# indrajeetadityaroy9/vit-inductive-bias-distillation

Measured on AMD Instinct MI355X. Metric: distillation images/sec (BASD loss fwd+bwd+grad all-reduce), DeiT-S<-ResNet-50 @ bs256/GPU, higher is better.
Workload: dtype f32; 1 GPU; cfg2 DeiT-S<-ResNet-50 224x224; per_gpu_batch=256, global_batch=256, input_dtype=float32, layout=strided (CLS-sliced / channel-major views), backward=True, grad_allreduce_bytes=88202672, grad_allreduce=none at world size 1 (bucket packed, nothing to exchange), rank_readback=auto, readback_deferred_steps=1756, selector=basd_selector_chain mode 0, parallelism=dp1

## Files before the change

### include/basd_hip.h

```cpp
#ifndef BASD_HIP_H
#define BASD_HIP_H

#include <stdint.h>

#ifdef __cplusplus
extern "C" {
#endif

#ifndef __HIP_PLATFORM_AMD__
typedef struct ihipStream_t* hipStream_t;
#endif

#define BASD_OK 0
#define BASD_EINVAL (-1)
#define BASD_EUNSUPPORTED (-2)
#define BASD_DTYPE_F32 0
#define BASD_DTYPE_BF16 1
#define BASD_DTYPE_U8 2


int basd_gemm_nt(const void* a, int a_dtype, long a_sb, long a_sn, long a_sd, int a_rows_per_batch,
                 long a_batch_stride, const float* b, long ldb, long b_batch_stride, int M, int N, int K, int batch,
                 float* c, long ldc, long c_batch_stride, float scale, const float* bias, float beta,
                 float* colsum_part, float* col_mean, hipStream_t stream);

int basd_gemm_tn_splits(int krows);

int basd_gemm_tn(const void* a, const void* b, int dtype, long a_sb, long a_sn, long a_sd, long a_batch_stride,
                 long b_sb, long b_sn, long b_sd, long b_batch_stride, int rows_per_batch, int krows, int M, int N,
                 int batch, const float* mean_a, const float* mean_b, int splits, float* slabs, float* c, long ldc,
                 long c_batch_stride, float scale, hipStream_t stream);

int basd_colmean_parts(int rows);

int basd_colmean(const void* x, int dtype, long sb, long sn, long sd, int rows_per_batch, long batch_stride,
                 int rows, int cols, int batch, int parts, float* partial, float* mean, hipStream_t stream);

int basd_gemm_tuning(int split_bf16);
int basd_gemm_tuning_get(void);

int basd_colmean_multi(const void* const* x_ptrs, int dtype, long sb, long sn, long sd, int rows_per_batch, int rows,
                       int cols, int n_mats, int parts, float* partial, float* means, int vec_ok,
                       hipStream_t stream);

int basd_syrk_splits(int krows, int cols, int n_mats);

int basd_syrk_multi(const void* const* x_ptrs, int dtype, long sb, long sn, long sd, int rows_per_batch, int krows,
                    int cols, int n_mats, const float* means, const float* scales, int splits, float* slabs,
                    float* out, long out_stride, int vec_ok, const float* fold, int fold_parts, int fold_from,
                    hipStream_t stream);


int basd_jacobi_workspace_ints(int batch, int max_sweeps);
int basd_jacobi_max_rows(void);
int basd_jacobi_plain4_fits(int n);

int basd_jacobi_tuning(int lanes_per_pair);
int basd_jacobi_ordering(int odd_even);

int basd_jacobi_onesided(float* W, long batch_stride, int rows_dot, int rows_tot, int n, int batch,
                         const int* n_arr, float* colnorm, int colnorm_stride, int max_sweeps, float tol_cos,
                         int* flags, int* sweeps_out, hipStream_t stream);
int basd_jacobi_plan_query(int rows_dot, int rows_tot, int n, int batch, int per_matrix_orders, int* out8);

long basd_jacobi_twopass_workspace_bytes(int n, int batch, int max_sweeps);
int basd_jacobi_stacked_twopass(float* W, long batch_stride, int n, int batch, float* colnorm, int colnorm_stride,
                                int max_sweeps, float tol_cos, void* workspace, int* sweeps_out, hipStream_t stream);

int basd_sort_extract(const float* W, long batch_stride, int rows, int rows_tot, int n, int batch,
                      const float* colnorm, int colnorm_stride, float* vals_desc, float* vecs, int kmax,
                      hipStream_t stream);


long basd_tridiag_workspace_bytes(int n, int batch);

int basd_tridiag(float* a, long a_batch_stride, int n, int batch, float* d, float* e, float* tau, float* vh,
                 void* work, hipStream_t stream);

int basd_tridiag_ranked(float* a, long a_batch_stride, int n, int batch, float* d, float* e, float* tau, float* vh,
                        void* work, int rank_count, double factor, int cap, int* rank_out, int* host_mirror,
                        void* mid_event ,
                        hipStream_t stream);

// ... 410 lines not shown
```

### vit-inductive-bias-distillation_amd/basd_amd/_lib.py

```python
from __future__ import annotations

import ctypes as C
import os
import threading

_HERE = os.path.dirname(os.path.abspath(__file__))
LIB_PATH = os.path.join(_HERE, "libbasd_hip.so")

vp, i32, i64, f32, f64 = C.c_void_p, C.c_int, C.c_long, C.c_float, C.c_double

SIGNATURES = {
    "basd_gemm_nt": [vp, i32, i64, i64, i64, i32, i64, vp, i64, i64, i32, i32, i32, i32, vp, i64, i64, f32, vp, f32,
                     vp, vp, vp],
    "basd_gemm_tn_splits": [i32],
    "basd_gemm_tn": [vp, vp, i32, i64, i64, i64, i64, i64, i64, i64, i64, i32, i32, i32, i32, i32, vp, vp, i32, vp,
                     vp, i64, i64, f32, vp],
    "basd_colmean_parts": [i32],
    "basd_colmean": [vp, i32, i64, i64, i64, i32, i64, i32, i32, i32, i32, vp, vp, vp],
    "basd_colmean_multi": [vp, i32, i64, i64, i64, i32, i32, i32, i32, i32, vp, vp, i32, vp],
    "basd_syrk_splits": [i32, i32, i32],
    "basd_syrk_multi": [vp, i32, i64, i64, i64, i32, i32, i32, i32, vp, vp, i32, vp, vp, i64, i32, vp, i32, i32, vp],
    "basd_jacobi_workspace_ints": [i32, i32],
    "basd_jacobi_max_rows": [],
    "basd_jacobi_twopass_workspace_bytes": [i32, i32, i32],
    "basd_jacobi_stacked_twopass": [vp, i64, i32, i32, vp, i32, i32, f32, vp, vp, vp],
    "basd_jacobi_tuning": [i32],
    "basd_jacobi_ordering": [i32],
    "basd_gemm_tuning": [i32],
    "basd_gemm_tuning_get": [],
    "basd_jacobi_onesided": [vp, i64, i32, i32, i32, i32, vp, vp, i32, i32, f32, vp, vp, vp],
    "basd_jacobi_plan_query": [i32, i32, i32, i32, i32, vp],
    "basd_sort_extract": [vp, i64, i32, i32, i32, i32, vp, i32, vp, vp, i32, vp],
    "basd_tridiag_workspace_bytes": [i32, i32],
    "basd_tridiag_tuning": [i32, i32, i32, i32, i32, i32],
    "basd_tridiag": [vp, i64, i32, i32, vp, vp, vp, vp, vp, vp],
    "basd_tridiag_ranked": [vp, i64, i32, i32, vp, vp, vp, vp, vp, i32, f64, i32, vp, vp, vp, vp],
    "basd_tridiag_ranked_gated": [vp, i64, i32, i32, vp, vp, vp, vp, vp, i32, f64, i32, vp, vp, vp, C.c_uint, i32, vp],
    "basd_flag_set": [vp, C.c_uint, vp],
    "basd_scale_unless_one": [vp, i64, vp, vp, vp],
    "basd_event_create": [vp],
    "basd_event_destroy": [vp],
    "basd_stream_wait_event": [vp, vp],
    "basd_tridiag_eigenvalues": [vp, vp, i32, i32, vp, vp],
    "basd_tridiag_eigenvalues_leading": [vp, vp, i32, i32, i32, vp, vp],
    "basd_tridiag_apply_q": [vp, vp, i32, i32, i32, vp, vp, i32, i32, vp],
    "basd_tridiag_shifted_solve": [vp, vp, vp, i32, i32, i32, i32, vp, vp, vp],
    "basd_tridiag_mp_rank": [vp, vp, i32, i32, f64, i32, vp, vp, vp, vp, vp],
    "basd_tridiag_mp_rank_rank1": [vp, vp, vp, i32, i32, f64, f64, i32, vp, vp, vp, vp],
    "basd_tridiag_eigenvectors": [vp, vp, vp, vp, vp, i32, i32, i32, vp, vp, i32, vp],
    "basd_mp_rank": [vp, i32, i32, f64, i32, vp, vp, vp],
    "basd_grassmann_distance": [vp, i32, vp, vp, i32, vp, i32, vp, vp, vp],
    "basd_grassmann_distance_padded": [vp, i32, i32, vp, vp, i32, vp, i32, vp, vp],
    "basd_selector_tail": [vp] * 10 + [i32, i32, i32, i32] + [vp] * 14 + [vp],
    "basd_sqrt_clamp": [vp, vp, i64, vp],
# ... 164 lines not shown
```

### vit-inductive-bias-distillation_amd/csrc/chain.hip

```cpp
#include "basd_common.h"
#include "../../include/basd_hip.h"
#include <stdlib.h>

namespace basd {

__global__ void __launch_bounds__(256) chain_sw_kernel(const float* __restrict__ vals, int n, int kmax,
                                                       float* __restrict__ sw) {
    const int l = blockIdx.x;
    for (int i = threadIdx.x; i < kmax; i += 256) sw[(long)l * kmax + i] = sqrtf(fmaxf(vals[(long)l * n + i], 0.f));
}

__global__ void chain_k_arr_kernel(const int* __restrict__ ranks, int L, int items, int kmax, int* __restrict__ k_arr) {
    const int i = blockIdx.x * blockDim.x + threadIdx.x;
    if (i < items) {
        int k = ranks[i % L];
        k = k < 1 ? 1 : k;
        k_arr[i] = k > kmax ? kmax : k;
    }
}

constexpr int CERT_BLOCKS = 32;
__global__ void __launch_bounds__(256) rank_certificate_kernel(const float* __restrict__ grams, const float* __restrict__ zbar,
                                                               int n, int L, double factor, double* __restrict__ scratch,
                                                               int* __restrict__ host_flag) {
    __shared__ double part[2][4];
    __shared__ int s_last;
    const int tid = threadIdx.x, lane = tid & 63, wave = tid >> 6, l = blockIdx.y;
    const long nn = (long)n * n;
    const float* g = grams + l * nn;
    double s2 = 0.0, tr = 0.0;
    for (long idx = (long)blockIdx.x * 256 + tid; idx < nn; idx += (long)CERT_BLOCKS * 256) {
        const double v = (double)g[idx];
        s2 = fma(v, v, s2);
    }
    if (blockIdx.x == 0)
        for (int i = tid; i < n; i += 256) tr += (double)g[(long)i * n + i];
    for (int off = 32; off > 0; off >>= 1) {
        s2 += __shfl_down(s2, off, 64);
        tr += __shfl_down(tr, off, 64);
    }
    if (lane == 0) { part[0][wave] = s2; part[1][wave] = tr; }
    __syncthreads();
    int* ticket = (int*)(scratch + 4L * L);
    if (tid == 0) {
        atomicAdd(scratch + 4 * l + 0, part[0][0] + part[0][1] + part[0][2] + part[0][3]);
        if (blockIdx.x == 0) atomicAdd(scratch + 4 * l + 1, part[1][0] + part[1][1] + part[1][2] + part[1][3]);
        __threadfence();
        s_last = atomicAdd(ticket, 1) == CERT_BLOCKS * L - 1;
    }
    __syncthreads();
    if (!s_last) return;
    __threadfence();
    __shared__ int s_ok;
    if (tid == 0) s_ok = 1;
    __syncthreads();
    for (int m = wave; m < L; m += 4) {
        double zz = 0.0;
        if (zbar)
            for (int i = lane; i < n; i += 64) {
                const double z = (double)zbar[(long)m * n + i];
                zz = fma(z, z, zz);
            }
        for (int off = 32; off > 0; off >>= 1) zz += __shfl_down(zz, off, 64);
        if (lane == 0) {
            const double a = __hip_atomic_load(scratch + 4 * m + 0, __ATOMIC_RELAXED, __HIP_MEMORY_SCOPE_AGENT);
            const double b = __hip_atomic_load(scratch + 4 * m + 1, __ATOMIC_RELAXED, __HIP_MEMORY_SCOPE_AGENT);
            const double c = (double)(n - (n - 1) / 2);
            bool good = false;
            if (b > 0.0 && c > 1.0) {
                const double lo = fmax(zz, a / b);
                const double tr_a = fmax(b - zz, 1e-4 * b);
                const double hi = fmin(b / c, tr_a / (c - 1.0));
                good = lo > 1.5 * factor * hi;
            }
            if (!good) atomicAnd(&s_ok, 0);
            scratch[4 * m + 0] = 0.0;
            scratch[4 * m + 1] = 0.0;
        }
    }
    __syncthreads();
    if (tid == 0) {
        *ticket = 0;
        *host_flag = s_ok;
        __threadfence_system();
    }
}

__global__ void __launch_bounds__(256) chain_mask_cos_kernel(float* __restrict__ cos, int kmax, const int* __restrict__ k_arr) {
    const int k = k_arr[blockIdx.x];
    float* c = cos + (long)blockIdx.x * kmax * kmax;
    for (int idx = threadIdx.x; idx < kmax * kmax; idx += 256) {
        const int i = idx / kmax, j = idx - i * kmax;
        if (i >= k || j >= k) c[idx] = 0.f;
    }
// ... 131 lines not shown
    if (M_t < n || M_t > 0x7fffffff || M_s > 0x7fffffff) return BASD_EUNSUPPORTED;
    const long nn = (long)n * n;
    const int tiles = (int)((M_t + 127) / 128);
    hipStream_t cs = a->chain_stream, ss = a->student_stream;

    if (a->main_stream) BASD_HIP(hipEventRecord((hipEvent_t)a->ev_fork, a->main_stream));
    BASD_HIP(hipStreamWaitEvent(cs, (hipEvent_t)a->ev_fork, 0));
    if (ss != cs) BASD_HIP(hipStreamWaitEvent(ss, (hipEvent_t)a->ev_fork, 0));
    if (a->ev_slot_free) {
        BASD_HIP(hipStreamWaitEvent(cs, (hipEvent_t)a->ev_slot_free, 0));
        if (ss != cs) BASD_HIP(hipStreamWaitEvent(ss, (hipEvent_t)a->ev_slot_free, 0));
    }

    const bool early = mode == 3 && a->go_flag != nullptr && a->fact_stream != nullptr && a->go_value != 0;
    if (early) {
        hipStream_t fs = a->fact_stream;
        if (a->ev_slot_free) BASD_HIP(hipStreamWaitEvent(fs, (hipEvent_t)a->ev_slot_free, 0));
        int rc_early = basd_tridiag_ranked_gated(a->grams, nn, n, 2 * L, a->d, a->e, a->tau, a->vh, a->tri_work, L,
                                                 a->mp_factor, (int)a->rank_cap, a->ranks, a->host_mirror, a->go_flag,
                                                 (unsigned)a->go_value, (int)a->go_budget, fs);
        if (rc_early != BASD_OK) return rc_early;
        BASD_HIP(hipEventRecord((hipEvent_t)a->ev_ranks, fs));
    }
    for (int l = 0; l < L; ++l)
        BASD_TRY(basd_gemm_nt(a->teacher_host_ptrs[l], (int)a->t_dtype, a->t_sb, a->t_sn, a->t_sd, n_t, 0, a->proj_t, d_t,
                              0, (int)M_t, n, d_t, 1, a->z + (long)l * M_t * n, n, M_t * n, 1.f, nullptr, 0.f,
                              a->z_sums + (long)l * tiles * n, a->z_means + (long)l * n, cs));
    BASD_MARK(a->tm_proj, cs);
    if (mode == 4) {
        BASD_CHECK_ARG(a->ev_tgram != nullptr && ss != cs);
        BASD_HIP(hipEventRecord((hipEvent_t)a->ev_tgram, cs));
        BASD_HIP(hipStreamWaitEvent(ss, (hipEvent_t)a->ev_tgram, 0));
    }
    BASD_TRY(basd_syrk_multi(a->z_ptrs, BASD_DTYPE_F32, 0, n, 1, 1 << 30, (int)M_t, n, L, a->z_means, nullptr,
                             (int)a->t_splits, a->t_slabs, a->grams + (long)L * nn, nn, 1, nullptr, 0, 0, cs));
    BASD_TRY(basd_gram_finish(a->grams + (long)L * nn, a->z_means, n, L, M_t, a->grams, nullptr, cs));
    BASD_MARK(a->tm_tgram, cs);
    if (mode == 3) BASD_CHECK_ARG(a->ev_tg0 != nullptr);
    if (a->ev_tg0) BASD_HIP(hipEventRecord((hipEvent_t)a->ev_tg0, cs));
    if (a->cert_mirror) {
        BASD_CHECK_ARG(a->cert_stream && a->ev_cert && a->ev_tg0 && a->cert_scratch);
        if (a->cert_stream != cs) BASD_HIP(hipStreamWaitEvent(a->cert_stream, (hipEvent_t)a->ev_tg0, 0));
        BASD_TRY(basd_rank_certificate(a->grams, a->z_means, n, L, a->mp_factor, a->cert_scratch, a->cert_mirror, a->cert_stream));
        BASD_HIP(hipEventRecord((hipEvent_t)a->ev_cert, a->cert_stream));
    }

    auto student_grams = [&](hipStream_t st) -> int {
        BASD_MARK(a->tm_scol0, st);
        BASD_TRY(basd_colmean_multi(a->student_ptrs, (int)a->s_dtype, a->s_sb, a->s_sn, a->s_sd, n_s, (int)M_s, n, E,
                                    (int)a->s_parts, a->s_partial, a->s_means, (int)a->s_vec_ok, st));
        BASD_MARK(a->tm_scol1, st);
        BASD_TRY(basd_syrk_multi(a->student_ptrs, (int)a->s_dtype, a->s_sb, a->s_sn, a->s_sd, n_s, (int)M_s, n, E,
                                 a->s_means, nullptr, (int)a->s_splits, a->s_slabs, a->grams + 2L * L * nn, nn,
                                 (int)a->s_vec_ok, nullptr, 0, 0, st));
        BASD_MARK(a->tm_sgram, st);
        return BASD_OK;
    };

    if (mode == 0 || mode == 4) {
        BASD_TRY(student_grams(ss));
        if (ss != cs) {
            BASD_HIP(hipEventRecord((hipEvent_t)a->ev_student, ss));
            BASD_HIP(hipStreamWaitEvent(cs, (hipEvent_t)a->ev_student, 0));
        }
        BASD_MARK(a->tm_tri0, cs);
        BASD_TRY(basd_tridiag_ranked(a->grams, nn, n, 2 * L + E, a->d, a->e, a->tau, a->vh, a->tri_work, L, a->mp_factor,
                                     (int)a->rank_cap, a->ranks, a->host_mirror, a->tm_mid, cs));
        BASD_HIP(hipEventRecord((hipEvent_t)a->ev_ranks, cs));
    } else {
// ... 26 lines not shown
```

### vit-inductive-bias-distillation_amd/csrc/gemm.hip

```cpp
#include <type_traits>

#include "basd_common.h"

namespace basd {

typedef float f32x16 __attribute__((ext_vector_type(16)));
typedef float f32x4 __attribute__((ext_vector_type(4)));

template <typename T>
using lds_ptr = const __attribute__((address_space(3))) T*;

constexpr int BM = 128, BN = 128;

typedef __bf16 bf16x8 __attribute__((ext_vector_type(8)));

__device__ __forceinline__ unsigned cvt_pk_bf16(float a, float b) {
    unsigned r;
    asm("v_cvt_pk_bf16_f32 %0, %1, %2" : "=v"(r) : "v"(a), "v"(b));
    return r;
}

__device__ __forceinline__ void split3(float a, float b, unsigned& hi, unsigned& mid, unsigned& lo) {
    hi = cvt_pk_bf16(a, b);
    const float ra = a - __uint_as_float(hi << 16), rb = b - __uint_as_float(hi & 0xffff0000u);
// ... 646 lines not shown
    syrk_grid_decode(splits * n_mats, pairs, pair, unit);
    int tmi, tni;
    tri_tile(pair, tmi, tni);
    const bool diag = tmi == tni;
    lds_t* tA = lds;
    lds_t* tB = diag ? lds : lds + Path::TN_TILE;
    const int tid = threadIdx.x, lane = tid & 63, wave = tid >> 6, wm = wave >> 1, wn = wave & 1;
    const int m0 = tmi * BM, n0 = tni * BN;
    const int z = unit / splits, sp = unit - z * splits;
    X.ptr = ptrs[z];
    const float* mean = means ? means + (long)z * cols : nullptr;
    float* C = slabs + ((long)z * splits + sp) * (long)cols * cols;
    int k_begin, k_end;
    tn_split_range(Krows, splits, sp, k_begin, k_end);

    f32x16 acc[2][2];
    zero_acc(acc);

    const bool is_b = tid >= 128;
    const bool loader = !(is_b && diag);
    const int t = tid & 127;
    const int col0 = is_b ? n0 : m0;
    float m4[4];
    TnCursor cu;
    tn_cursor_init(cu, X, k_begin, t);
    if (fold && z >= fold_from)
        tn_fold_mean4(fold + (long)(z - fold_from) * fold_parts * cols, fold_parts, cols, Krows, col0, t, m4);
    else
        tn_mean4(mean, cols, col0, t, m4);
    tn_main_loop<Path, T, VEC>(X, cu, loader, k_begin, k_end, cols, col0, t, m4, is_b ? tB : tA, tA, tB, wm, wn, lane, acc);
    Path::tn_store_c(C, cols, cols, cols, m0, n0, acc, wm, wn, lane, 1.f);
}

__global__ void __launch_bounds__(256) syrk_reduce_kernel(const float* __restrict__ slabs, int cols, int splits,
                                                          const float* __restrict__ scales, float* __restrict__ out,
                                                          long out_stride) {
    int tmi, tni;
    tri_tile(blockIdx.x >> 6, tmi, tni);
    const int e = (blockIdx.x & 63) * 256 + threadIdx.x;
    const int r = tmi * BM + (e >> 7), c = tni * BN + (e & 127);
    if (r >= cols || c >= cols) return;
    const int z = blockIdx.y;
    const long mat = (long)cols * cols;
    const bool up = tmi == tni && r < c;
    const float* in = slabs + (long)z * splits * mat + (up ? (long)c * cols + r : (long)r * cols + c);
    float s = 0.f;
    for (int k = 0; k < splits; ++k) s += in[k * mat];
    s *= scales ? scales[z] : 1.f;
    float* o = out + (long)z * out_stride;
    o[(long)r * cols + c] = s;
    if (tmi != tni) o[(long)c * cols + r] = s;
}

__global__ void reduce_slabs_kernel(const float* __restrict__ slabs, long slab_stride, int splits, long count,
                                    float scale, float* __restrict__ out, long batch_in_stride,
                                    long batch_out_stride) {
    const float* in = slabs + (long)blockIdx.y * batch_in_stride;
    float* o = out + (long)blockIdx.y * batch_out_stride;
    for (long i = (long)blockIdx.x * blockDim.x + threadIdx.x; i < count; i += (long)gridDim.x * blockDim.x) {
        float s = 0.f;
        for (int k = 0; k < splits; ++k) s += in[(long)k * slab_stride + i];
        o[i] = s * scale;
    }
}

template <typename T>
__global__ void __launch_bounds__(256) colsum_partial_kernel(GemmOperand X, int rows, int cols, int parts,
                                                             float* __restrict__ partial,
                                                             const void* const* __restrict__ ptrs = nullptr) {
    __shared__ float red[4][64];
    const int cl = threadIdx.x & 63, rg = threadIdx.x >> 6, c = blockIdx.x * 64 + cl;
    const T* base = ptrs ? (const T*)ptrs[blockIdx.z] : (const T*)X.ptr + (long)blockIdx.z * X.batch_stride;
    const int per = (rows + parts - 1) / parts;
    const int r0 = blockIdx.y * per, r1 = min(rows, r0 + per);
    float s = 0.f;
    if (c < cols)
        for (int r = r0 + rg; r < r1; r += 4) s += to_f32(base[row_off(X, r) + (long)c * X.sd]);
    red[rg][cl] = s;
    __syncthreads();
    if (rg == 0 && c < cols)
        partial[((long)blockIdx.z * parts + blockIdx.y) * cols + c] = (red[0][cl] + red[1][cl]) + (red[2][cl] + red[3][cl]);
}

__device__ __forceinline__ float4 load4(const float* p) { return *(const float4*)p; }
// ... 192 lines not shown
    BASD_CHECK_ARG(x && partial && mean && rows > 0 && cols > 0 && batch > 0 && parts >= 1);
    GemmOperand X{x, sb, sn, sd, rows_per_batch, batch_stride};
    const int esz = dtype == BASD_DTYPE_F32 ? 4 : 2;
    const bool vec = sd == 1 && cols % 4 == 0 && ((uintptr_t)x & 15) == 0 && (sb * esz) % 16 == 0 &&
                     (sn * esz) % 16 == 0 && (batch_stride * esz) % 16 == 0;
    if (dtype == BASD_DTYPE_F32) launch_colsum<float>(X, nullptr, x, rows, cols, parts, batch, vec, partial, stream);
    else if (dtype == BASD_DTYPE_BF16) launch_colsum<__hip_bfloat16>(X, nullptr, x, rows, cols, parts, batch, vec, partial, stream);
    else return BASD_EINVAL;
    colsum_final_kernel<<<dim3((cols + 63) / 64, batch), 256, 0, stream>>>(partial, cols, parts, 1.f / rows, mean);
    BASD_RETURN_LAST();
}

int basd_syrk_splits(int krows, int cols, int n_mats) {
    const int tiles = (cols + BM - 1) / BM, pairs = tiles * (tiles + 1) / 2;
    const long w = (long)pairs * n_mats;
    const int chunks = (krows + TN_BK - 1) / TN_BK;
    int cap = chunks / 8;
    if (cap > 64) cap = 64;
    if (cap < 1) cap = 1;
    const double slots = 768.0;
    auto fill = [&](int s) {
        const double x = (double)(w * s) / slots;
        const double rounds = x <= 1.0 ? 1.0 : (double)(long)(x + 0.999999);
        return x / rounds;
    };
    double best_eff = 0.0;
    for (int s = 1; s <= cap; ++s) best_eff = fill(s) > best_eff ? fill(s) : best_eff;
    int best = cap;
    for (int s = 1; s <= cap; ++s)
        if (fill(s) >= 0.97 * best_eff) { best = s; break; }
    return best;
}

int basd_syrk_multi(const void* const* x_ptrs, int dtype, long sb, long sn, long sd, int rows_per_batch, int krows,
                    int cols, int n_mats, const float* means, const float* scales, int splits, float* slabs,
                    float* out, long out_stride, int vec_ok, const float* fold, int fold_parts, int fold_from,
                    hipStream_t stream) {
    BASD_CHECK_ARG(x_ptrs && slabs && out && krows > 0 && cols > 0 && n_mats > 0 && splits >= 1 && rows_per_batch > 0);
    BASD_CHECK_ARG(out_stride >= (long)cols * cols);
    BASD_CHECK_ARG(!fold || (fold_parts > 0 && fold_from >= 0 && fold_from <= n_mats));
    GemmOperand X{nullptr, sb, sn, sd, rows_per_batch, 0};
    const int tiles = (cols + BM - 1) / BM, pairs = tiles * (tiles + 1) / 2;
    const dim3 grid(pairs * splits * n_mats);
    const bool vec = dtype == BASD_DTYPE_F32 ? vec_ok && sd == 1 && sb % 4 == 0 && sn % 4 == 0 : sd == 1;
    const bool known = dispatch_mfma(g_gemm_split, dtype, vec, [&](auto path, auto el, auto v) {
        syrk_tn_kernel<decltype(path), typename decltype(el)::type, decltype(v)::value><<<grid, 256, 0, stream>>>(
            x_ptrs, X, cols, krows, splits, n_mats, pairs, means, slabs, fold, fold_parts, fold_from);
    });
    if (!known) return BASD_EINVAL;
    syrk_reduce_kernel<<<dim3(pairs * 64, n_mats), 256, 0, stream>>>(slabs, cols, splits, scales, out, out_stride);
    BASD_RETURN_LAST();
}

int basd_colmean_multi(const void* const* x_ptrs, int dtype, long sb, long sn, long sd, int rows_per_batch, int rows,
                       int cols, int n_mats, int parts, float* partial, float* means, int vec_ok,
                       hipStream_t stream) {
    BASD_CHECK_ARG(x_ptrs && partial && means && rows > 0 && cols > 0 && n_mats > 0 && parts >= 1);
    GemmOperand X{nullptr, sb, sn, sd, rows_per_batch, 0};
    const int esz = dtype == BASD_DTYPE_F32 ? 4 : 2;
    const bool vec = vec_ok && sd == 1 && cols % 4 == 0 && (sb * esz) % 16 == 0 && (sn * esz) % 16 == 0;
    if (dtype == BASD_DTYPE_F32) launch_colsum<float>(X, x_ptrs, nullptr, rows, cols, parts, n_mats, vec, partial, stream);
    else if (dtype == BASD_DTYPE_BF16) launch_colsum<__hip_bfloat16>(X, x_ptrs, nullptr, rows, cols, parts, n_mats, vec, partial, stream);
    else return BASD_EINVAL;
    colsum_final_kernel<<<dim3((cols + 63) / 64, n_mats), 256, 0, stream>>>(partial, cols, parts, 1.f / rows, means);
    BASD_RETURN_LAST();
}

}
```

### vit-inductive-bias-distillation_amd/csrc/procrustes.hip

```cpp
#include "basd_common.h"
#include "../../include/basd_hip.h"

namespace basd {

typedef double f64x4 __attribute__((ext_vector_type(4)));

template <typename T>
__global__ void __launch_bounds__(256) token_weights_kernel(const void* const* __restrict__ attn_ptrs,
                                                            const float* __restrict__ mix, int L, long sb, long sh,
                                                            long sq, long sk, int H, int A, int has_cls, int n_a,
                                                            int n_t, int n_s, const int* __restrict__ atap0,
                                                            const int* __restrict__ atap1,
                                                            const float* __restrict__ alam,
                                                            const int* __restrict__ tap0,
                                                            const int* __restrict__ tap1,
                                                            const float* __restrict__ lam, float* __restrict__ omega,
                                                            float* __restrict__ omega_t, float* __restrict__ raw_out) {
    extern __shared__ float sm[];
    float* raw = sm;
    float* w = sm + n_a;
    __shared__ float red[32];
    const int b = blockIdx.x, tid = threadIdx.x;
    for (int j = tid; j < n_a; j += blockDim.x) {
        float acc = 0.f;
        if (has_cls) {
            for (int h = 0; h < H; ++h) {
                float m = 0.f;
                for (int l = 0; l < L; ++l)
                    m += mix[l] * ldg_f32((const BASD_GLOBAL_AS T*)attn_ptrs[l] + (b * sb + h * sh + (long)(1 + j) * sk));
                acc += m;
            }
            acc /= (float)H;
        } else {
            for (int h = 0; h < H; ++h)
                for (int q = 0; q < A; ++q) {
                    float m = 0.f;
                    for (int l = 0; l < L; ++l)
                        m += mix[l] * ldg_f32((const BASD_GLOBAL_AS T*)attn_ptrs[l] + (b * sb + h * sh + q * sq + (long)j * sk));
                    acc += m;
                }
            acc /= (float)(H * A);
        }
        raw[j] = acc;
        if (raw_out) raw_out[(long)b * n_a + j] = acc;
    }
    __syncthreads();
    float part = 0.f;
    for (int n = tid; n < n_s; n += blockDim.x) {
        float v;
        if (atap0) {
            const float l1 = alam[n];
            v = (1.f - l1) * raw[atap0[n]] + l1 * raw[atap1[n]];
        } else {
            v = raw[n];
        }
        w[n] = v;
        part += v;
    }
    const float total = block_sum(part, red);
    for (int n = tid; n < n_s; n += blockDim.x) {
        const float v = w[n] / total;
        w[n] = v;
        omega[(long)b * n_s + n] = v;
    }
    __syncthreads();
    for (int j = tid; j < n_t; j += blockDim.x) {
        float acc = 0.f;
        if (tap0) {
            for (int n = 0; n < n_s; ++n) {
                const float l1 = lam[n];
                if (tap0[n] == j) acc += (1.f - l1) * w[n];
                if (tap1[n] == j) acc += l1 * w[n];
            }
        } else {
            acc = w[j];
        }
        omega_t[(long)b * n_t + j] = acc;
    }
}

template <typename T>
__global__ void __launch_bounds__(256) student_project_kernel(const T* __restrict__ X, long sb, long sn, int n_s,
                                                              int n_t, int D, const float* __restrict__ omega,
                                                              const int* __restrict__ tap0,
                                                              const int* __restrict__ tap1,
                                                              const float* __restrict__ lam,
                                                              const int* __restrict__ range0,
                                                              const int* __restrict__ range1,
                                                              float* __restrict__ mu_out, float* __restrict__ tr_part,
                                                              float* __restrict__ Ap) {
    extern __shared__ float sm[];
    float* w = sm;
    __shared__ float red[4][64];
    __shared__ float mu[64];
    __shared__ float scratch[32];
    const int b = blockIdx.y, d0 = blockIdx.x * 64, tid = threadIdx.x;
    const int cl = tid & 63, rg = tid >> 6, d = d0 + cl;
    const bool live = d < D;
    const T* Xb = X + (long)b * sb + d;
    for (int n = tid; n < n_s; n += 256) w[n] = omega[(long)b * n_s + n];
    __syncthreads();
    float acc = 0.f;
    if (live)
        for (int n = rg; n < n_s; n += 4) acc = fmaf(w[n], to_f32(Xb[(long)n * sn]), acc);
    red[rg][cl] = acc;
// ... 168 lines not shown
    if (tid < SP_W) {
        float m = 0.f;
#pragma unroll
        for (int q = 0; q < 32; ++q) m += red[q][tid];
        mu[tid] = m;
        if (d0 + tid < D) mu_out[((long)e * B + b) * D + d0 + tid] = m;
    }
    __syncthreads();
    const float4 m4 = *(const float4*)(mu + c4);
    float part = 0.f;
    if (live)
        for (int n = rg; n < n_s; n += 32) {
            const float4 v = *(const float4*)(xs + n * SP_W + c4);
            const float cx = v.x - m4.x, cy = v.y - m4.y, cz = v.z - m4.z, cw = v.w - m4.w;
            part = fmaf(w[n], fmaf(cx, cx, fmaf(cy, cy, fmaf(cz, cz, cw * cw))), part);
        }
    const float tr = block_sum(part, scratch);
    if (tid == 0) tr_part[((long)e * B + b) * gridDim.x + blockIdx.x] = tr;
    if (!live) return;
    float* Ab = Ap + ((long)e * B + b) * n_t * D + d0 + c4;
    for (int j = rg; j < n_t; j += 32) {
        const int n0 = range0 ? range0[j] : j, n1 = range1 ? range1[j] : j + 1;
        float4 a = make_float4(0.f, 0.f, 0.f, 0.f);
        for (int n = n0; n < n1; ++n) {
            const float cw = tap0 ? (t0[n] == j ? c0[n] : 0.f) + (t1[n] == j ? c1[n] : 0.f) : w[n];
            const float4 v = *(const float4*)(xs + n * SP_W + c4);
            a.x = fmaf(cw, v.x - m4.x, a.x); a.y = fmaf(cw, v.y - m4.y, a.y);
            a.z = fmaf(cw, v.z - m4.z, a.z); a.w = fmaf(cw, v.w - m4.w, a.w);
        }
        *(float4*)(Ab + (long)j * D) = a;
    }
}

template <typename T>
__global__ void __launch_bounds__(256) teacher_center_kernel(const void* const* __restrict__ tok_ptrs,
                                                             const float* __restrict__ mix, int L, long sb, long sn,
                                                             long sd, int n, int D, const int* __restrict__ g0,
                                                             const int* __restrict__ g1,
                                                             const float* __restrict__ glam,
                                                             const float* __restrict__ omega_t,
                                                             float* __restrict__ mu_out, float* __restrict__ Tc) {
    extern __shared__ float sm[];
    float* tile = sm;
    float* wt = sm + (size_t)n * 65;
    float* mu = wt + n;
    const int b = blockIdx.y, d0 = blockIdx.x * 64, tid = threadIdx.x;
    for (int j = tid; j < n; j += 256) wt[j] = omega_t[(long)b * n + j];
    const int total = n * 64;
    const bool feat_fast = sd == 1;
    for (int idx = tid; idx < total; idx += 256) {
        int j, dd;
        if (feat_fast) { j = idx >> 6; dd = idx & 63; }
        else { dd = idx / n; j = idx - dd * n; }
        const int d = d0 + dd;
        float v = 0.f;
        if (d < D) {
            const long off = b * sb + (long)d * sd;
            if (g0) {
                const long r0 = g0[j], r1 = g1[j];
                float a0 = 0.f, a1 = 0.f;
                for (int l = 0; l < L; ++l) {
                    const BASD_GLOBAL_AS T* p = (const BASD_GLOBAL_AS T*)tok_ptrs[l];
                    a0 = fmaf(mix[l], ldg_f32(p + (off + r0 * sn)), a0);
                    a1 = fmaf(mix[l], ldg_f32(p + (off + r1 * sn)), a1);
                }
                const float l1 = glam[j];
                v = (1.f - l1) * a0 + l1 * a1;
            } else {
                for (int l = 0; l < L; ++l)
                    v = fmaf(mix[l], ldg_f32((const BASD_GLOBAL_AS T*)tok_ptrs[l] + (off + (long)j * sn)), v);
            }
        }
        tile[j * 65 + dd] = v;
    }
    __syncthreads();
    if (tid < 64) {
        float acc = 0.f;
        for (int j = 0; j < n; ++j) acc = fmaf(wt[j], tile[j * 65 + tid], acc);
        mu[tid] = acc;
        if (d0 + tid < D) mu_out[(long)b * D + d0 + tid] = acc;
    }
    __syncthreads();
    float* out = Tc + (long)b * n * D;
    for (int idx = tid; idx < total; idx += 256) {
        const int j = idx >> 6, dd = idx & 63, d = d0 + dd;
        if (d < D) out[(long)j * D + d] = tile[j * 65 + dd] - mu[dd];
    }
}

constexpr int TCM_W = 16, TCM_G = 4;
template <typename T>
__global__ void __launch_bounds__(256) teacher_center_multi_kernel(
    const void* const* __restrict__ tok_ptrs, const float* __restrict__ mix, int L, int G, long sb, long sn, long sd,
    int n, int D, const int* __restrict__ g0, const int* __restrict__ g1, const float* __restrict__ glam,
    const float* __restrict__ omega_t, float* __restrict__ mu_out, float* __restrict__ Tc) {
    extern __shared__ float sm[];
    const int B = gridDim.y, b = blockIdx.y, d0 = blockIdx.x * TCM_W, tid = threadIdx.x;
    float* tile = sm;
    float* wt = sm + (size_t)G * n * (TCM_W + 1);
    float* mu = wt + (size_t)G * n;
    for (int idx = tid; idx < G * n; idx += 256) {
        const int g = idx / n, j = idx - g * n;
        wt[idx] = omega_t[((long)g * B + b) * n + j];
    }
    const int total = n * TCM_W;
    const bool feat_fast = sd == 1;
    for (int idx = tid; idx < total; idx += 256) {
// ... 945 lines not shown
                                                                      const int* __restrict__ tap0,
                                                                      const int* __restrict__ tap1,
                                                                      const float* __restrict__ lam,
                                                                      const int* __restrict__ range0,
                                                                      const int* __restrict__ range1,
                                                                      float* __restrict__ dX) {
    const int j = blockIdx.x, b = blockIdx.y;
    const int s0 = range0[j], s1 = range1[j];
    for (int d = threadIdx.x; d < D; d += 128) {
        float acc = 0.f;
        for (int s = s0; s < s1; ++s) {
            const float l1 = lam[s];
            const float coef = (tap0[s] == j ? 1.f - l1 : 0.f) + (tap1[s] == j ? l1 : 0.f);
            acc = fmaf(coef, dY[((long)b * n_out + s) * D + d], acc);
        }
        dX[((long)b * n_in + j) * D + d] = acc;
    }
}

}

using namespace basd;

extern "C" {

int basd_token_weights(const void* const* attn_ptrs, int dtype, const float* mix, int L, long sb, long sh, long sq,
                       long sk, int B, int H, int A, int has_cls, int n_a, int n_t, int n_s, const int* atap0,
                       const int* atap1, const float* alam, const int* tap0, const int* tap1, const float* lam,
                       float* omega, float* omega_t, float* raw_out, hipStream_t stream) {
    BASD_CHECK_ARG(attn_ptrs && mix && omega && omega_t && L > 0 && B > 0 && H > 0 && n_a > 0 && n_t > 0 && n_s > 0);
    BASD_CHECK_ARG(A == n_a + (has_cls ? 1 : 0));
    BASD_CHECK_ARG((n_a == n_s) == (atap0 == nullptr));
    BASD_CHECK_ARG((n_t == n_s) == (tap0 == nullptr));
    const size_t lds = sizeof(float) * (size_t)(n_a + n_s);
    if (dtype == BASD_DTYPE_F32)
        token_weights_kernel<float><<<B, 256, lds, stream>>>(attn_ptrs, mix, L, sb, sh, sq, sk, H, A, has_cls, n_a, n_t, n_s, atap0, atap1, alam, tap0, tap1, lam, omega, omega_t, raw_out);
    else if (dtype == BASD_DTYPE_BF16)
        token_weights_kernel<__hip_bfloat16><<<B, 256, lds, stream>>>(attn_ptrs, mix, L, sb, sh, sq, sk, H, A, has_cls, n_a, n_t, n_s, atap0, atap1, alam, tap0, tap1, lam, omega, omega_t, raw_out);
    else
        return BASD_EINVAL;
    BASD_RETURN_LAST();
}

int basd_student_project(const void* x, int dtype, long sb, long sn, int B, int n_s, int n_t, int D,
                         const float* omega, const int* tap0, const int* tap1, const float* lam, const int* range0,
                         const int* range1, float* mu, float* tr_s, float* a_prime, hipStream_t stream) {
    BASD_CHECK_ARG(x && omega && mu && tr_s && a_prime && B > 0 && n_s > 0 && n_t > 0 && D > 0);
    BASD_CHECK_ARG((n_t == n_s) == (tap0 == nullptr));
    const size_t lds = sizeof(float) * (size_t)n_s;
    const dim3 grid((D + 63) / 64, B);
    const int esz = dtype == BASD_DTYPE_F32 ? 4 : 2;
    const size_t lds_slab = sizeof(float) * (size_t)n_s * 65;
    const bool staged = D % 4 == 0 && ((uintptr_t)x * 1) % 16 == 0 && (sb * esz) % 16 == 0 && (sn * esz) % 16 == 0 &&
                        (esz == 4 || D % 8 == 0) && lds_slab <= 64 * 1024;
    if (dtype == BASD_DTYPE_F32) {
        if (staged) {
            (void)hipFuncSetAttribute((const void*)student_project_lds_kernel<float>, hipFuncAttributeMaxDynamicSharedMemorySize, (int)lds_slab);
            student_project_lds_kernel<float><<<grid, 256, lds_slab, stream>>>((const float*)x, sb, sn, n_s, n_t, D, omega, tap0, tap1, lam, range0, range1, mu, tr_s, a_prime);
        } else {
            student_project_kernel<float><<<grid, 256, lds, stream>>>((const float*)x, sb, sn, n_s, n_t, D, omega, tap0, tap1, lam, range0, range1, mu, tr_s, a_prime);
        }
    } else if (dtype == BASD_DTYPE_BF16) {
        if (staged) {
            (void)hipFuncSetAttribute((const void*)student_project_lds_kernel<__hip_bfloat16>, hipFuncAttributeMaxDynamicSharedMemorySize, (int)lds_slab);
            student_project_lds_kernel<__hip_bfloat16><<<grid, 256, lds_slab, stream>>>((const __hip_bfloat16*)x, sb, sn, n_s, n_t, D, omega, tap0, tap1, lam, range0, range1, mu, tr_s, a_prime);
        } else {
            student_project_kernel<__hip_bfloat16><<<grid, 256, lds, stream>>>((const __hip_bfloat16*)x, sb, sn, n_s, n_t, D, omega, tap0, tap1, lam, range0, range1, mu, tr_s, a_prime);
// ... 383 lines not shown
```

Measured before the change: 175,600 images/s.

## Batch independent loads in reduction kernels and fuse gram finish into syrk reduce

Several kernels now issue a batch of independent global loads before accumulating: the rank certificate reduction, the syrk slab reduce, token weights, and the teacher-center tile fill. The goal is more memory-level parallelism in loops that are bound by load latency. The syrk reduce can also write the uncentered gram directly, which removes the separate gram_finish launch and its extra read of the grams. Token weights now stage the tap and lambda arrays in LDS, and the teacher-center fill gains a 32-bit offset path. The cost is higher register pressure and more template variants.

```diff
diff --git a/include/basd_hip.h b/include/basd_hip.h
--- a/include/basd_hip.h
+++ b/include/basd_hip.h
@@ -49,6 +49,10 @@
                     int cols, int n_mats, const float* means, const float* scales, int splits, float* slabs,
                     float* out, long out_stride, int vec_ok, const float* fold, int fold_parts, int fold_from,
                     hipStream_t stream);
+int basd_syrk_multi_finish(const void* const* x_ptrs, int dtype, long sb, long sn, long sd, int rows_per_batch,
+                           int krows, int cols, int n_mats, const float* means, const float* scales, int splits,
+                           float* slabs, float* out, long out_stride, int vec_ok, const float* fold, int fold_parts,
+                           int fold_from, const float* zbar, long m_rows, float* out_u, hipStream_t stream);
 
 
 int basd_jacobi_workspace_ints(int batch, int max_sweeps);
diff --git a/vit-inductive-bias-distillation_amd/basd_amd/_lib.py b/vit-inductive-bias-distillation_amd/basd_amd/_lib.py
--- a/vit-inductive-bias-distillation_amd/basd_amd/_lib.py
+++ b/vit-inductive-bias-distillation_amd/basd_amd/_lib.py
@@ -20,6 +20,8 @@
     "basd_colmean_multi": [vp, i32, i64, i64, i64, i32, i32, i32, i32, i32, vp, vp, i32, vp],
     "basd_syrk_splits": [i32, i32, i32],
     "basd_syrk_multi": [vp, i32, i64, i64, i64, i32, i32, i32, i32, vp, vp, i32, vp, vp, i64, i32, vp, i32, i32, vp],
+    "basd_syrk_multi_finish": [vp, i32, i64, i64, i64, i32, i32, i32, i32, vp, vp, i32, vp, vp, i64, i32, vp, i32, i32,
+                               vp, i64, vp, vp],
     "basd_jacobi_workspace_ints": [i32, i32],
     "basd_jacobi_max_rows": [],
     "basd_jacobi_twopass_workspace_bytes": [i32, i32, i32],
diff --git a/vit-inductive-bias-distillation_amd/csrc/chain.hip b/vit-inductive-bias-distillation_amd/csrc/chain.hip
--- a/vit-inductive-bias-distillation_amd/csrc/chain.hip
+++ b/vit-inductive-bias-distillation_amd/csrc/chain.hip
@@ -19,7 +19,7 @@
     }
 }
 
-constexpr int CERT_BLOCKS = 32;
+constexpr int CERT_BLOCKS = 32, CERT_BATCH = 8;
 __global__ void __launch_bounds__(256) rank_certificate_kernel(const float* __restrict__ grams, const float* __restrict__ zbar,
                                                                int n, int L, double factor, double* __restrict__ scratch,
                                                                int* __restrict__ host_flag) {
@@ -29,9 +29,17 @@
     const long nn = (long)n * n;
     const float* g = grams + l * nn;
     double s2 = 0.0, tr = 0.0;
-    for (long idx = (long)blockIdx.x * 256 + tid; idx < nn; idx += (long)CERT_BLOCKS * 256) {
-        const double v = (double)g[idx];
-        s2 = fma(v, v, s2);
+    constexpr long stride = (long)CERT_BLOCKS * 256;
+    for (long idx = (long)blockIdx.x * 256 + tid; idx < nn; idx += CERT_BATCH * stride) {
+        float v[CERT_BATCH];
+#pragma unroll
+        for (int u = 0; u < CERT_BATCH; ++u) v[u] = g[idx + u * stride < nn ? idx + u * stride : idx];
+#pragma unroll
+        for (int u = 0; u < CERT_BATCH; ++u)
+            if (idx + u * stride < nn) {
+                const double d = (double)v[u];
+                s2 = fma(d, d, s2);
+            }
     }
     if (blockIdx.x == 0)
         for (int i = tid; i < n; i += 256) tr += (double)g[(long)i * n + i];
@@ -57,9 +65,16 @@
     for (int m = wave; m < L; m += 4) {
         double zz = 0.0;
         if (zbar)
-            for (int i = lane; i < n; i += 64) {
-                const double z = (double)zbar[(long)m * n + i];
-                zz = fma(z, z, zz);
+            for (int i = lane; i < n; i += 64 * CERT_BATCH) {
+                float v[CERT_BATCH];
+#pragma unroll
+                for (int u = 0; u < CERT_BATCH; ++u) v[u] = zbar[(long)m * n + (i + 64 * u < n ? i + 64 * u : i)];
+#pragma unroll
+                for (int u = 0; u < CERT_BATCH; ++u)
+                    if (i + 64 * u < n) {
+                        const double z = (double)v[u];
+                        zz = fma(z, z, zz);
+                    }
             }
         for (int off = 32; off > 0; off >>= 1) zz += __shfl_down(zz, off, 64);
         if (lane == 0) {
@@ -257,9 +272,9 @@
         BASD_HIP(hipEventRecord((hipEvent_t)a->ev_tgram, cs));
         BASD_HIP(hipStreamWaitEvent(ss, (hipEvent_t)a->ev_tgram, 0));
     }
-    BASD_TRY(basd_syrk_multi(a->z_ptrs, BASD_DTYPE_F32, 0, n, 1, 1 << 30, (int)M_t, n, L, a->z_means, nullptr,
-                             (int)a->t_splits, a->t_slabs, a->grams + (long)L * nn, nn, 1, nullptr, 0, 0, cs));
-    BASD_TRY(basd_gram_finish(a->grams + (long)L * nn, a->z_means, n, L, M_t, a->grams, nullptr, cs));
+    BASD_TRY(basd_syrk_multi_finish(a->z_ptrs, BASD_DTYPE_F32, 0, n, 1, 1 << 30, (int)M_t, n, L, a->z_means, nullptr,
+                                    (int)a->t_splits, a->t_slabs, a->grams + (long)L * nn, nn, 1, nullptr, 0, 0,
+                                    a->z_means, M_t, a->grams, cs));
     BASD_MARK(a->tm_tgram, cs);
     if (mode == 3) BASD_CHECK_ARG(a->ev_tg0 != nullptr);
     if (a->ev_tg0) BASD_HIP(hipEventRecord((hipEvent_t)a->ev_tg0, cs));
diff --git a/vit-inductive-bias-distillation_amd/csrc/gemm.hip b/vit-inductive-bias-distillation_amd/csrc/gemm.hip
--- a/vit-inductive-bias-distillation_amd/csrc/gemm.hip
+++ b/vit-inductive-bias-distillation_amd/csrc/gemm.hip
@@ -702,9 +702,12 @@
     Path::tn_store_c(C, cols, cols, cols, m0, n0, acc, wm, wn, lane, 1.f);
 }
 
+constexpr int RED_BATCH = 16;
+template <bool FINISH>
 __global__ void __launch_bounds__(256) syrk_reduce_kernel(const float* __restrict__ slabs, int cols, int splits,
                                                           const float* __restrict__ scales, float* __restrict__ out,
-                                                          long out_stride) {
+                                                          long out_stride, const float* __restrict__ zbar,
+                                                          float m_rows, float* __restrict__ out_u) {
     int tmi, tni;
     tri_tile(blockIdx.x >> 6, tmi, tni);
     const int e = (blockIdx.x & 63) * 256 + threadIdx.x;
@@ -714,12 +717,27 @@
     const long mat = (long)cols * cols;
     const bool up = tmi == tni && r < c;
     const float* in = slabs + (long)z * splits * mat + (up ? (long)c * cols + r : (long)r * cols + c);
+    float zr = 0.f, zc = 0.f;
+    if (FINISH) { zr = zbar[(long)z * cols + r]; zc = zbar[(long)z * cols + c]; }
     float s = 0.f;
-    for (int k = 0; k < splits; ++k) s += in[k * mat];
+    constexpr int NB = FINISH ? RED_BATCH : 1;
+    for (int k0 = 0; k0 < splits; k0 += NB) {
+        float v[NB];
+#pragma unroll
+        for (int u = 0; u < NB; ++u) v[u] = in[min(k0 + u, splits - 1) * mat];
+#pragma unroll
+        for (int u = 0; u < NB; ++u)
+            if (k0 + u < splits) s += v[u];
+    }
     s *= scales ? scales[z] : 1.f;
     float* o = out + (long)z * out_stride;
     o[(long)r * cols + c] = s;
     if (tmi != tni) o[(long)c * cols + r] = s;
+    if (FINISH) {
+        float* ou = out_u + (long)z * mat;
+        ou[(long)r * cols + c] = fmaf(m_rows * zr, zc, s) / m_rows;
+        if (tmi != tni) ou[(long)c * cols + r] = fmaf(m_rows * zc, zr, s) / m_rows;
+    }
 }
 
 __global__ void reduce_slabs_kernel(const float* __restrict__ slabs, long slab_stride, int splits, long count,
@@ -978,10 +996,10 @@
     return best;
 }
 
-int basd_syrk_multi(const void* const* x_ptrs, int dtype, long sb, long sn, long sd, int rows_per_batch, int krows,
-                    int cols, int n_mats, const float* means, const float* scales, int splits, float* slabs,
-                    float* out, long out_stride, int vec_ok, const float* fold, int fold_parts, int fold_from,
-                    hipStream_t stream) {
+static int syrk_multi(const void* const* x_ptrs, int dtype, long sb, long sn, long sd, int rows_per_batch, int krows,
+                      int cols, int n_mats, const float* means, const float* scales, int splits, float* slabs,
+                      float* out, long out_stride, int vec_ok, const float* fold, int fold_parts, int fold_from,
+                      const float* zbar, long m_rows, float* out_u, hipStream_t stream) {
     BASD_CHECK_ARG(x_ptrs && slabs && out && krows > 0 && cols > 0 && n_mats > 0 && splits >= 1 && rows_per_batch > 0);
     BASD_CHECK_ARG(out_stride >= (long)cols * cols);
     BASD_CHECK_ARG(!fold || (fold_parts > 0 && fold_from >= 0 && fold_from <= n_mats));
@@ -994,8 +1012,29 @@
             x_ptrs, X, cols, krows, splits, n_mats, pairs, means, slabs, fold, fold_parts, fold_from);
     });
     if (!known) return BASD_EINVAL;
-    syrk_reduce_kernel<<<dim3(pairs * 64, n_mats), 256, 0, stream>>>(slabs, cols, splits, scales, out, out_stride);
+    const dim3 rgrid(pairs * 64, n_mats);
+    if (out_u)
+        syrk_reduce_kernel<true><<<rgrid, 256, 0, stream>>>(slabs, cols, splits, scales, out, out_stride, zbar, (float)m_rows, out_u);
+    else
+        syrk_reduce_kernel<false><<<rgrid, 256, 0, stream>>>(slabs, cols, splits, scales, out, out_stride, nullptr, 0.f, nullptr);
     BASD_RETURN_LAST();
+}
+
+int basd_syrk_multi(const void* const* x_ptrs, int dtype, long sb, long sn, long sd, int rows_per_batch, int krows,
+                    int cols, int n_mats, const float* means, const float* scales, int splits, float* slabs,
+                    float* out, long out_stride, int vec_ok, const float* fold, int fold_parts, int fold_from,
+                    hipStream_t stream) {
+    return syrk_multi(x_ptrs, dtype, sb, sn, sd, rows_per_batch, krows, cols, n_mats, means, scales, splits, slabs, out,
+                      out_stride, vec_ok, fold, fold_parts, fold_from, nullptr, 0, nullptr, stream);
+}
+
+int basd_syrk_multi_finish(const void* const* x_ptrs, int dtype, long sb, long sn, long sd, int rows_per_batch,
+                           int krows, int cols, int n_mats, const float* means, const float* scales, int splits,
+                           float* slabs, float* out, long out_stride, int vec_ok, const float* fold, int fold_parts,
+                           int fold_from, const float* zbar, long m_rows, float* out_u, hipStream_t stream) {
+    BASD_CHECK_ARG(zbar && out_u && m_rows > 0);
+    return syrk_multi(x_ptrs, dtype, sb, sn, sd, rows_per_batch, krows, cols, n_mats, means, scales, splits, slabs, out,
+                      out_stride, vec_ok, fold, fold_parts, fold_from, zbar, m_rows, out_u, stream);
 }
 
 int basd_colmean_multi(const void* const* x_ptrs, int dtype, long sb, long sn, long sd, int rows_per_batch, int rows,
diff --git a/vit-inductive-bias-distillation_amd/csrc/procrustes.hip b/vit-inductive-bias-distillation_amd/csrc/procrustes.hip
--- a/vit-inductive-bias-distillation_amd/csrc/procrustes.hip
+++ b/vit-inductive-bias-distillation_amd/csrc/procrustes.hip
@@ -5,6 +5,7 @@
 
 typedef double f64x4 __attribute__((ext_vector_type(4)));
 
+constexpr int TW_BATCH = 16;
 template <typename T>
 __global__ void __launch_bounds__(256) token_weights_kernel(const void* const* __restrict__ attn_ptrs,
                                                             const float* __restrict__ mix, int L, long sb, long sh,
@@ -19,28 +20,51 @@
     extern __shared__ float sm[];
     float* raw = sm;
     float* w = sm + n_a;
+    float* lam_s = w + n_s;
+    int* tap0_s = (int*)(lam_s + n_s);
+    int* tap1_s = tap0_s + n_s;
     __shared__ float red[32];
     const int b = blockIdx.x, tid = threadIdx.x;
+    if (tap0)
+        for (int n = tid; n < n_s; n += blockDim.x) { lam_s[n] = lam[n]; tap0_s[n] = tap0[n]; tap1_s[n] = tap1[n]; }
+    const int Q = has_cls ? 1 : A, rows = H * Q;
     for (int j = tid; j < n_a; j += blockDim.x) {
+        const long col = b * sb + (long)(has_cls ? 1 + j : j) * sk;
         float acc = 0.f;
-        if (has_cls) {
-            for (int h = 0; h < H; ++h) {
-                float m = 0.f;
-                for (int l = 0; l < L; ++l)
-                    m += mix[l] * ldg_f32((const BASD_GLOBAL_AS T*)attn_ptrs[l] + (b * sb + h * sh + (long)(1 + j) * sk));
-                acc += m;
-            }
-            acc /= (float)H;
-        } else {
-            for (int h = 0; h < H; ++h)
-                for (int q = 0; q < A; ++q) {
-                    float m = 0.f;
-                    for (int l = 0; l < L; ++l)
-                        m += mix[l] * ldg_f32((const BASD_GLOBAL_AS T*)attn_ptrs[l] + (b * sb + h * sh + q * sq + (long)j * sk));
-                    acc += m;
+        int h = 0, q = 0;
+        for (int r0 = 0; r0 < rows; r0 += TW_BATCH) {
+            long off[TW_BATCH];
+#pragma unroll
+            for (int u = 0; u < TW_BATCH; ++u) {
+                off[u] = r0 + u < rows ? col + h * sh + q * sq : col;
+                if (++q == Q) { q = 0; ++h; }
+            }
+            float m[TW_BATCH];
+            if (L == 1) {
+                const BASD_GLOBAL_AS T* p = (const BASD_GLOBAL_AS T*)attn_ptrs[0];
+                const float mix0 = mix[0];
+                float v[TW_BATCH];
+#pragma unroll
+                for (int u = 0; u < TW_BATCH; ++u) v[u] = ldg_f32(p + off[u]);
+#pragma unroll
+                for (int u = 0; u < TW_BATCH; ++u) { m[u] = 0.f; m[u] += mix0 * v[u]; }
+            } else {
+#pragma unroll
+                for (int u = 0; u < TW_BATCH; ++u) m[u] = 0.f;
+                for (int l = 0; l < L; ++l) {
+                    const BASD_GLOBAL_AS T* p = (const BASD_GLOBAL_AS T*)attn_ptrs[l];
+                    float v[TW_BATCH];
+#pragma unroll
+                    for (int u = 0; u < TW_BATCH; ++u) v[u] = ldg_f32(p + off[u]);
+#pragma unroll
+                    for (int u = 0; u < TW_BATCH; ++u) m[u] += mix[l] * v[u];
                 }
-            acc /= (float)(H * A);
-        }
+            }
+#pragma unroll
+            for (int u = 0; u < TW_BATCH; ++u)
+                if (r0 + u < rows) acc += m[u];
+        }
+        acc /= (float)rows;
         raw[j] = acc;
         if (raw_out) raw_out[(long)b * n_a + j] = acc;
     }
@@ -68,9 +92,9 @@
         float acc = 0.f;
         if (tap0) {
             for (int n = 0; n < n_s; ++n) {
-                const float l1 = lam[n];
-                if (tap0[n] == j) acc += (1.f - l1) * w[n];
-                if (tap1[n] == j) acc += l1 * w[n];
+                const float l1 = lam_s[n];
+                if (tap0_s[n] == j) acc += (1.f - l1) * w[n];
+                if (tap1_s[n] == j) acc += l1 * w[n];
             }
         } else {
             acc = w[j];
@@ -305,6 +329,94 @@
     }
 }
 
+constexpr int TC_BATCH = 16, TC_BATCH_G = 4;
+
+template <bool NARROW> struct tc_off { typedef long type; };
+template <> struct tc_off<true> { typedef unsigned type; };
+template <typename T, int NB, bool GATHER, bool FEAT, bool NARROW>
+__device__ __forceinline__ void tc_fill(const void* const* __restrict__ tok_ptrs, const float* __restrict__ mix, int L,
+                                        long sb, long sn, long sd, int n, int D, const int* __restrict__ g0,
+                                        const int* __restrict__ g1, const float* __restrict__ glam, int b, int d0,
+                                        int tid, float* tile) {
+    const int total = n * 64;
+    const int step_dd = 256 / n, step_j = 256 - step_dd * n;
+    typedef typename tc_off<NARROW>::type off_t;
+    static_assert(!(NARROW && GATHER), "gathered rows have no span known here");
+    const long base = b * sb + (long)d0 * sd;
+    auto load = [&](const BASD_GLOBAL_AS T* p, off_t o) {
+        if (NARROW) return ldg_f32((const BASD_GLOBAL_AS T*)((const BASD_GLOBAL_AS char*)(p + base) + o));
+        return ldg_f32(p + o);
+    };
+    int dd_cm = tid / n, j_cm = tid - dd_cm * n;
+    auto next = [&](int idx, int& j, int& dd) {
+        if (FEAT) { j = idx >> 6; dd = idx & 63; }
+        else {
+            dd = dd_cm; j = j_cm;
+            dd_cm += step_dd; j_cm += step_j;
+            if (j_cm >= n) { j_cm -= n; ++dd_cm; }
+        }
+    };
+    for (int idx0 = tid; idx0 < total; idx0 += 256 * NB) {
+        const int dd_trip = dd_cm, j_trip = j_cm;
+        off_t o0[NB], o1[NB];
+        float l1[NB];
+#pragma unroll
+        for (int u = 0; u < NB; ++u) {
+            const int idx = idx0 + 256 * u;
+            int j, dd;
+            next(idx, j, dd);
+            const bool live = idx < total && d0 + dd < D;
+            const int js = live ? j : 0;
+            const long off = (NARROW ? 0 : base) + (long)(live ? dd : 0) * sd;
+            if (GATHER) {
+                o0[u] = (off_t)(off + (long)g0[js] * sn);
+                o1[u] = (off_t)(off + (long)g1[js] * sn);
+                l1[u] = glam[js];
+            } else {
+                o0[u] = NARROW ? (off_t)((off + (long)js * sn) * (long)sizeof(T)) : (off_t)(off + (long)js * sn);
+            }
+        }
+        float v[NB];
+        if (GATHER) {
+            float a0[NB], a1[NB];
+#pragma unroll
+            for (int u = 0; u < NB; ++u) a0[u] = a1[u] = 0.f;
+            for (int l = 0; l < L; ++l) {
+                const BASD_GLOBAL_AS T* p = (const BASD_GLOBAL_AS T*)tok_ptrs[l];
+                float x0[NB], x1[NB];
+#pragma unroll
+                for (int u = 0; u < NB; ++u) { x0[u] = load(p, o0[u]); x1[u] = load(p, o1[u]); }
+#pragma unroll
+                for (int u = 0; u < NB; ++u) {
+                    a0[u] = fmaf(mix[l], x0[u], a0[u]);
+                    a1[u] = fmaf(mix[l], x1[u], a1[u]);
+                }
+            }
+#pragma unroll
+            for (int u = 0; u < NB; ++u) v[u] = (1.f - l1[u]) * a0[u] + l1[u] * a1[u];
+        } else {
+#pragma unroll
+            for (int u = 0; u < NB; ++u) v[u] = 0.f;
+            for (int l = 0; l < L; ++l) {
+                const BASD_GLOBAL_AS T* p = (const BASD_GLOBAL_AS T*)tok_ptrs[l];
+                float x[NB];
+#pragma unroll
+                for (int u = 0; u < NB; ++u) x[u] = load(p, o0[u]);
+#pragma unroll
+                for (int u = 0; u < NB; ++u) v[u] = fmaf(mix[l], x[u], v[u]);
+            }
+        }
+        dd_cm = dd_trip; j_cm = j_trip;
+#pragma unroll
+        for (int u = 0; u < NB; ++u) {
+            const int idx = idx0 + 256 * u;
+            int j, dd;
+            next(idx, j, dd);
+            if (idx < total) tile[j * 65 + dd] = d0 + dd < D ? v[u] : 0.f;
+        }
+    }
+}
+
 template <typename T>
 __global__ void __launch_bounds__(256) teacher_center_kernel(const void* const* __restrict__ tok_ptrs,
                                                              const float* __restrict__ mix, int L, long sb, long sn,
@@ -321,31 +433,20 @@
     for (int j = tid; j < n; j += 256) wt[j] = omega_t[(long)b * n + j];
     const int total = n * 64;
     const bool feat_fast = sd == 1;
-    for (int idx = tid; idx < total; idx += 256) {
-        int j, dd;
-        if (feat_fast) { j = idx >> 6; dd = idx & 63; }
-        else { dd = idx / n; j = idx - dd * n; }
-        const int d = d0 + dd;
-        float v = 0.f;
-        if (d < D) {
-            const long off = b * sb + (long)d * sd;
-            if (g0) {
-                const long r0 = g0[j], r1 = g1[j];
-                float a0 = 0.f, a1 = 0.f;
-                for (int l = 0; l < L; ++l) {
-                    const BASD_GLOBAL_AS T* p = (const BASD_GLOBAL_AS T*)tok_ptrs[l];
-                    a0 = fmaf(mix[l], ldg_f32(p + (off + r0 * sn)), a0);
-                    a1 = fmaf(mix[l], ldg_f32(p + (off + r1 * sn)), a1);
-                }
-                const float l1 = glam[j];
-                v = (1.f - l1) * a0 + l1 * a1;
-            } else {
-                for (int l = 0; l < L; ++l)
-                    v = fmaf(mix[l], ldg_f32((const BASD_GLOBAL_AS T*)tok_ptrs[l] + (off + (long)j * sn)), v);
-            }
-        }
-        tile[j * 65 + dd] = v;
-    }
+    const bool narrow = sd >= 0 && sn >= 0 && (63 * sd + (n - 1) * sn) * (long)sizeof(T) < (1L << 31);
+#define BASD_TC_FILL(NB, GATHER, FEAT, NARROW) \
+    tc_fill<T, NB, GATHER, FEAT, NARROW>(tok_ptrs, mix, L, sb, sn, sd, n, D, g0, g1, glam, b, d0, tid, tile)
+    if (g0) {
+        if (feat_fast) BASD_TC_FILL(TC_BATCH_G, true, true, false);
+        else BASD_TC_FILL(TC_BATCH_G, true, false, false);
+    } else if (narrow) {
+        if (feat_fast) BASD_TC_FILL(TC_BATCH, false, true, true);
+        else BASD_TC_FILL(TC_BATCH, false, false, true);
+    } else {
+        if (feat_fast) BASD_TC_FILL(TC_BATCH_G, false, true, false);
+        else BASD_TC_FILL(TC_BATCH_G, false, false, false);
+    }
+#undef BASD_TC_FILL
     __syncthreads();
     if (tid < 64) {
         float acc = 0.f;
@@ -1357,7 +1458,12 @@
     BASD_CHECK_ARG(A == n_a + (has_cls ? 1 : 0));
     BASD_CHECK_ARG((n_a == n_s) == (atap0 == nullptr));
     BASD_CHECK_ARG((n_t == n_s) == (tap0 == nullptr));
-    const size_t lds = sizeof(float) * (size_t)(n_a + n_s);
+    const size_t lds = sizeof(float) * ((size_t)n_a + (size_t)n_s * (tap0 ? 4 : 1));
+    if (lds > 150 * 1024) return BASD_EUNSUPPORTED;
+    if (lds > 48 * 1024) {
+        (void)hipFuncSetAttribute((const void*)token_weights_kernel<float>, hipFuncAttributeMaxDynamicSharedMemorySize, 150 * 1024);
+        (void)hipFuncSetAttribute((const void*)token_weights_kernel<__hip_bfloat16>, hipFuncAttributeMaxDynamicSharedMemorySize, 150 * 1024);
+    }
     if (dtype == BASD_DTYPE_F32)
         token_weights_kernel<float><<<B, 256, lds, stream>>>(attn_ptrs, mix, L, sb, sh, sq, sk, H, A, has_cls, n_a, n_t, n_s, atap0, atap1, alam, tap0, tap1, lam, omega, omega_t, raw_out);
     else if (dtype == BASD_DTYPE_BF16)
```

Result: no change. 175,900 images/s, median of 2 (+0.1%).
